# satoken/ractip

Measured on AMD Instinct MI355X. Metric: sequence-pairs/sec (incl. bp+hp+ap DP; host strings in, thresholded matrices out) at n=500, higher is better.
Workload: dtype f64; 1 GPU; synthetic random pairs n=500/500, std::mt19937(12345) stream (BASELINE config 3); scoring=CONTRAfold complementary (708 weights)

## Files before the change

### ractip_amd/csrc/compute.hip

```cpp
#include <hip/hip_runtime.h>

#include <algorithm>
#include <cmath>
#include <cstring>
#include <string>
#include <vector>

#include "ctx.h"
#include "kernels.h"

namespace rh::host {

template <class L, class... Args>
int run_graphed(rh_ctx* c, GraphSlot& g, hipStream_t stream, int k, L launcher, const Args&... args)
{
    const auto launch = [&] { int rc = RH_OK; ((rc = rc ? rc : launcher(c, args)), ...); return rc; };
    if (!c->use_graphs || c->time_cls >= 0) return launch();
    size_t key = 1469598103934665603ull + (sizeof(Args) + ...);
    const auto mix = [&](const void* p, size_t n) { for (size_t q = 0; q < n; q++) key = (key ^ ((const unsigned char*)p)[q]) * 0x100000001b3ull; };
    (mix(&args, sizeof(Args)), ...);
    int *launch_counter = &c->n_launch[k], *far_counter = &c->n_far[k];
    if (!g.exec || g.key != key) {
        if (g.exec) { HIP_TRY(c, hipGraphExecDestroy(g.exec)); g.exec = nullptr; }
        hipGraph_t graph = nullptr;
// ... 4 lines not shown
        if (rc) { if (graph) (void)hipGraphDestroy(graph); return rc; }
        if (e != hipSuccess) { if (graph) (void)hipGraphDestroy(graph); return fail(c, RH_ERR_HIP, "graph capture failed: %s", hipGetErrorString(e)); }
        e = hipGraphInstantiate(&g.exec, graph, nullptr, nullptr, 0);
        (void)hipGraphDestroy(graph);
        if (e != hipSuccess) { g.exec = nullptr; return fail(c, RH_ERR_HIP, "hipGraphInstantiate failed: %s", hipGetErrorString(e)); }
        g.key = key;
        g.launches = *launch_counter - before;
        g.far = *far_counter - far_before;
        *launch_counter = before;
        *far_counter = far_before;
    }
    HIP_TRY(c, hipGraphLaunch(g.exec, stream));
    *launch_counter += g.launches;
    *far_counter += g.far;
    return RH_OK;
}

McLinArgs mc_lin_args(const rh_ctx* c, int phase, const McBatch& B, const LinSet* lin, bool routed)
{
    McLinArgs A;
    A.B = B; A.lin = lin; A.phase = phase;
    A.logz = c->d_mclogz.as<double>(); A.bad = c->d_bad.as<int>();
    A.plan = plan_mc_lin(c, phase, B.nmax);
    if (routed && (!c->small_list.empty() || c->n_short > 0)) {
        A.routed = 1;
        A.small_list = c->d_small_list.as<const int>(); A.n_small = (int)c->small_list.size();
        A.n_sweep = c->d_n_sweep.as<const int>(); A.nmax_sweep = c->nmax_sweep;
        A.n_short = c->d_n_short.as<const int>(); A.nmax_short = c->nmax_short; A.short_count = c->n_short;
        A.plan_sweep = plan_mc_lin(c, phase, A.nmax_sweep);
        A.plan_short = plan_mc_lin(c, phase, A.nmax_short);
    }
    A.pin = xcd_pin(B.ns);
    A.strip_xcd = c->strip_xcd;
    A.f5_jlo = 32;
    A.up_w = c->max_w;
    A.f5_pass = c->f5_pass && f5_pass_fits(B.ld);
    return A;
}

static McVlinArgs mc_vlin_args(const rh_ctx* c, int phase, bool co)
{
    McVlinArgs A;
    A.B = co ? c->co : c->mc; A.phase = phase; A.co = co;
    A.pin = xcd_pin(A.B.ns);
    A.plan = plan_mc_vlin(c, phase, co, A.B.nmax);
    A.d_vlin = c->d_vlin; A.h_vlin = c->h_vlin; A.hplen = c->h_hplen.data(); A.d_hplen = c->d_hplen.as<const double>();
    A.bad = co ? c->d_cobad.as<int>() : c->d_bad.as<int>();
    if (co) {
        const DxBatch& D = c->dx;
        if (A.B.seeded) { A.from = c->mc; A.pair_seq = c->d_pidx.as<const int>(); }
        A.hp = D.hp; A.hp_logz = D.logz; A.hp_stride = D.tab_stride; A.hp_ldd = D.ldd; A.n1max = D.n1max; A.n2max = D.n2max;
        A.cut_min = c->co_cut_min; A.cut_max = c->co_cut_max;
        A.window = c->co_window && c->co_cut_min >= 1 && (phase == 1 || A.B.seeded);
    } else {
        A.logz = c->d_mclogz.as<double>(); A.gaps = c->d_gaps.as<double>(); A.max_w = c->max_w;
        A.acc_wide = c->acc_wide && (size_t)VM_COUNT * A.B.tab_stride * sizeof(double) < ((size_t)1 << 32);
        A.acc_final_t = c->acc_final_t && c->max_w <= 15;
    }
    return A;
}

static DxLinArgs dx_args(const rh_ctx* c)
{
    DxLinArgs A;
    A.X = c->dxl; A.plan = c->plan[2]; A.lz_chunks = c->lz_chunks;
    A.zpart = c->d_zpart.as<double>(); A.zbar = c->d_zbar.as<double>();
// ... 341 lines not shown
```

### ractip_amd/csrc/ctx.h

```cpp
#pragma once
#include <hip/hip_runtime.h>

#include <cassert>
#include <cstdint>
#include <cstring>
#include <string>
#include <type_traits>
#include <vector>

#include "../../include/ractip_hot.h"
#include "batch.h"
#include "batch_request.h"
#include "score_model.h"
#include "lin_model.h"
#include "vienna_model.h"
#include "scale_order.h"

struct rh_ctx;

namespace rh::host {

struct DevBuf {
    void* p = nullptr;
    size_t cap = 0;
// ... 36 lines not shown
};

struct SweepPlan {
    enum Org { kNone, kStrips, kPairs, kLookahead, kDiagonals, kDxStrip8, kDxSweep4, kDxSweepW };
    enum Far { kFarNone, kFarLds, kFarGather, kFarPacked };
    Org org = kNone;
    int W = 0;
    int BS = 0;
    int filt = 0;
    Far far = kFarNone;
    int far2_from = 0;
    int banded = 0;
    int repack2 = 0;
    const char* fine = "";
    const char* far_name = "";
};

static_assert(std::has_unique_object_representations_v<SweepPlan> && std::has_unique_object_representations_v<McBatch>);
static_assert(sizeof(DxLinBatch) == 4 * sizeof(void*) + 6 * sizeof(int) + 3 * sizeof(size_t) + 16 * sizeof(double), "no padding");

struct McLinArgs {
    McBatch B;
    const LinSet* lin;
    double* logz;
    int* bad;
    SweepPlan plan;
    const int* small_list;
    const int* n_sweep;
    const int* n_short;
    SweepPlan plan_sweep, plan_short;
    int routed, n_small, nmax_sweep, short_count, nmax_short;
    int phase, pin, strip_xcd;
    int f5_pass, f5_jlo;
    int up_w, pad_;
    McLinArgs() { std::memset(this, 0, sizeof *this); }
};

struct McVlinArgs {
    McBatch B;
    McBatch from;
    const int* pair_seq;
    SweepPlan plan;
    const VLinModel* d_vlin;
    const VLinModel* h_vlin;
    const double* hplen;
    const double* d_hplen;
    int* bad;
    double* logz;
    double* gaps;
    double* hp;
    double* hp_logz;
    size_t hp_stride;
    int hp_ldd, n1max, n2max;
    int window, cut_min, cut_max;
    int max_w, acc_wide, acc_final_t;
    int phase, pin, co;
    McVlinArgs() { std::memset(this, 0, sizeof *this); }
};

struct DxLinArgs {
    DxLinBatch X;
    SweepPlan plan;
    const DxLinModel* dm;
    const DxLinModel* hm;
    double vdx_s;
    double* zpart;
    double* zbar;
// ... 51 lines not shown
    DxLinModel h_dxlin;
    DevObj<DxLinModel> d_dxlin_r[4];
    DxLinModel h_dxlin_r[4];
    std::vector<int> rescaled_dx;
    DxLinBatch dxl = {};
    size_t dxl_layout = 0;
    size_t dx_bytes = 0;
    bool dxtab_log = false;
    int co_seed = 1;
    int dx_strip = 1;
    int dx_quad = 1;
    int dx_w = 4;
    int last_dx_path = 0;
    int far_mfma = 1;
    int lookahead = 2;
    int strip = 3;
    int far2 = -1;
    int strip_w = 8;
    int small_on = 0;
    std::vector<int> small_list;
    DevBuf d_small_list;
    DevBuf d_n_sweep;
    int nmax_sweep = 0;
    DevBuf d_n_short;
    int n_short = 0, nmax_short = 0;
    int strip_filt = 1;
    bool strip_filt_ok = false;
    int co_cut_min = 0, co_cut_max = 0;
    int co_window = 1;
    int acc_final_t = 1;
    int acc_wide = 1;
    int strip_xcd = 1;
    int f5_pass = 1;
    int far_pk = 1;
    int use_graphs = 1;
    GraphSlot g_in, g_out, g_dx;
    int mode = RH_MODE_AUTO;
    int duplex_mode = RH_MODE_INHERIT;
    int lin_w = 4;
    int lin_w_in = 4;
    int lin_bs = 16;
    int last_path = 0;
    bool last_went_log = false;
    SweepPlan plan[3];
    int max_w = 1;
    int region_acc = 0;
    DevBuf d_acc;
    hipEvent_t acc_ev[2] = {nullptr, nullptr};
    bool acc_timed = false;

    int np = 0, ns = 0;
    std::vector<int> pair_seq;
    std::vector<int> pair_seq_dev;
    bool indexed = false;
    bool has_mc = false, has_dx = false, computed = false;
    std::vector<int> n;
    McBatch mc = {};
    DxBatch dx = {};
    DevBuf d_seq;
    DevBuf d_n;
    DevBuf d_pseq;
    DevBuf d_pn;
    DevBuf d_pidx;
    DevBuf d_mctab;
    DevBuf d_corowp;
    DevBuf d_rowp;
// ... 148 lines not shown
```

### ractip_amd/csrc/kernels.h

```cpp
#pragma once
#include <hip/hip_runtime.h>

#include "../../include/ractip_hot.h"
#include "batch.h"
#include "score_model.h"
#include "lin_model.h"
#include "vienna_model.h"

namespace rh {
__global__ void mc_init(McBatch B);
__global__ void mc_inside_diag(McBatch B, const ScoreModel* __restrict__ M, int d, int pin);
__global__ void mc_outside_diag(McBatch B, const ScoreModel* __restrict__ M, int d, int pin);
__global__ void mc_unpaired(McBatch B, int max_w);
struct AccArgs {
    const LinModel* lin;
    const ScoreModel* score;
    double* scratch;
    int max_w, pad_;
};
constexpr int kAccTile = 64, kAccK = 16;
constexpr size_t acc_scratch_doubles(int ld) { return 3 * (size_t)ld * ld + 2 * 31 * (size_t)ld; }
template <int PATH> __global__ void cf_acc_hrows(McBatch B, AccArgs A);
template <int PATH> __global__ void cf_acc_hcols(McBatch B, AccArgs A);
template <int PATH> __global__ void cf_acc_gaps(McBatch B, AccArgs A);
template <int PATH> __global__ void cf_acc_final(McBatch B, AccArgs A);
template <int PATH> __global__ void cf_acc_sbuild(McBatch B, AccArgs A);
template <int PATH> __global__ void cf_acc_seed(McBatch B, AccArgs A);
template <int PATH> __global__ void cf_acc_link(McBatch B, AccArgs A, int flip);
template <int PATH> __global__ void cf_acc_close(McBatch B, AccArgs A, int j, int flip);
__global__ void dx_sweep_diag(DxBatch B, const ScoreModel* __restrict__ M, int t);
__global__ void dx_logz(DxBatch B, const ScoreModel* __restrict__ M);
__global__ void dx_posterior(DxBatch B);
__global__ void dx_hp_clear_rest(DxBatch B);
__global__ void lin_init(McBatch B, const LinModel* __restrict__ L, int* __restrict__ bad);
template <int W, int BS, int MODE> __global__ void lin_inside_diag(McBatch B, const LinModel* __restrict__ L, int d, double lam_d, int pin);
template <int W, int BS> __global__ void lin_outside_diag(McBatch B, const LinModel* __restrict__ L, int d, int pin, int* __restrict__ bad);
template <int W, int BS> __global__ void lin_outside_pair(McBatch B, const LinModel* __restrict__ L, int d, int khi, int pin, int* __restrict__ bad);
template <int BS> __global__ void lin_far_inside(McBatch B, int D);
template <int BS> __global__ void lin_far_outside(McBatch B, int D);
__global__ void lin_far_inside_mfma(McBatch B, int D);
__global__ void lin_far_outside_mfma(McBatch B, int D);
template <int SWEEP> __global__ void lin_pack_tiles(McBatch B, int Dblk, int outside, int banded);
template <int KD, int W, int FILT> __global__ void lin_inside_strip(McBatch B, const LinModel* __restrict__ L, const double* __restrict__ wT, int d0, double lam_d0, int pin);
template <int KD, int W, int FILT> __global__ void lin_outside_strip(McBatch B, const LinModel* __restrict__ L, const double* __restrict__ wT, int d0, int pin, int* __restrict__ bad);
__global__ void lin_f5i_tail(McBatch B, const LinModel* __restrict__ L, int jlo);
__global__ void lin_f5i_pass(McBatch B, const LinModel* __restrict__ L, int jlo);
void launch_lin_small(const McBatch& B, const LinModel* L, const double* wpad, const int* list, int nlist, int* bad, hipStream_t stream);
__global__ void lin_f5o_head(McBatch B, const LinModel* __restrict__ L, int khi, int klo);
__global__ void lin_f5o_pass(McBatch B, const LinModel* __restrict__ L);
__global__ void lin_far_inside_pk(McBatch B, int D, int l2);
__global__ void lin_far_outside_pk(McBatch B, int D, int l2);
__global__ void lin_far2_inside(McBatch B, int D2, int l2);
__global__ void lin_far2_outside(McBatch B, int D2, int l2);
__global__ void lin_finish(McBatch B, const LinModel* __restrict__ L, double* __restrict__ logz, int* __restrict__ bad);
template <int W> __global__ void dxl_sweep(DxLinBatch B, const DxLinModel* __restrict__ L, int step, int groups);
__global__ void dxl_sweep4(DxLinBatch B, const DxLinModel* __restrict__ L, int step, int groups);
__global__ void dxl_strip8(DxLinBatch B, const DxLinModel* __restrict__ L, int step);
template <bool S20> __global__ void dxvl_sweep4(DxLinBatch B, const VLinModel* __restrict__ L, const VDxLin* __restrict__ D, int step);
template <bool S20> __global__ void dxvl_logz_part(DxLinBatch B, const VLinModel* __restrict__ L, const VDxLin* __restrict__ D, double* __restrict__ zpart,
                               int* __restrict__ cpart, int nchunk);
__global__ void dxvl_logz_final(DxLinBatch B, double s, const double* __restrict__ zpart, const int* __restrict__ cpart, int nchunk,
                                double* __restrict__ zbar, double* __restrict__ logz, int* __restrict__ bad);
constexpr int kLzThreads = 256;
size_t dxl_logz_lds_bytes(int lds);
__global__ void dxl_logz_part(DxLinBatch B, const DxLinModel* __restrict__ L, double* __restrict__ zpart, int* __restrict__ cpart, int nchunk);
__global__ void dxl_logz_final(DxLinBatch B, const DxLinModel* __restrict__ L, const double* __restrict__ zpart, const int* __restrict__ cpart, int nchunk,
                               double* __restrict__ zbar, double* __restrict__ logz, int* __restrict__ bad);
__global__ void dxl_posterior(DxLinBatch B, const double* __restrict__ zbar, int* __restrict__ bad);
__global__ void dxv_sweep_diag(DxBatch B, const ViennaDx* __restrict__ V, int t);
__global__ void dxv_logz(DxBatch B, const ViennaDx* __restrict__ V);
__global__ void dxv_posterior(DxBatch B);
__global__ void mcv_init(McBatch B);
__global__ void mcv_inside_diag(McBatch B, const ViennaDx* __restrict__ V, int d, int pin);
__global__ void mcv_outside_diag(McBatch B, const ViennaDx* __restrict__ V, int d, int pin);
__global__ void mcv_acc_prep(McBatch B, const ViennaDx* __restrict__ V);
__global__ void mcv_acc_hscan(McBatch B, int slot);
__global__ void vlin_acc_prep(McBatch B, const VLinModel* __restrict__ L, const double* __restrict__ hplen);
// ... 71 lines not shown
```

### ractip_amd/csrc/launch_contrafold.hip

```cpp
#include <hip/hip_runtime.h>

#include <algorithm>
#include <cmath>
#include <cstring>
#include <string>
#include <vector>

#include "ctx.h"
#include "f5_stage.h"
#include "kernels.h"

__global__ void log_finish(rh::McBatch B, double* __restrict__ logz)
{
    const int sq = blockIdx.x * blockDim.x + threadIdx.x;
    if (sq < B.ns) logz[sq] = B.f5i[(size_t)sq * B.ld + B.n[sq]];
}

namespace rh::host {

int launch_mc_log(rh_ctx* c, int pin, const McBatch& B, double* logz_out)
{
    hipLaunchKernelGGL(mc_init, dim3((B.ns + 63) / 64), dim3(64), 0, c->s_mc, B);
    for (int d = 0; d <= B.nmax - 1; d++) {
        const int waves = std::max(B.nmax - 1 - d, 0) + 1;
// ... 71 lines not shown
#undef DIAG
#undef STRIP
static const DiagKernels& diag_kernels(int W, int BS) { return row_of(kDiag, [&](const DiagKernels& r) { return r.W == W && r.BS == BS; }); }
static const PairKernels& pair_kernels(int W) { return row_of(kOutsidePair, [&](const PairKernels& r) { return r.W == W; }); }
static const StripKernels& strip_kernels(int W, int filt) { return row_of(kStrip, [&](const StripKernels& r) { return r.W == W && r.filt == filt; }); }
static const LdsKernels& lds_kernels(int BS) { return row_of(kLds, [&](const LdsKernels& r) { return r.BS == BS; }); }

const char* far_name(SweepPlan::Far far, int BS, int phase)
{
    switch (far) {
        case SweepPlan::kFarLds: return phase == 0 ? lds_kernels(BS).in.name : lds_kernels(BS).out.name;
        case SweepPlan::kFarGather: return kFarGather[phase].name;
        case SweepPlan::kFarPacked: return kFarPacked[phase].name;
        default: return "";
    }
}
void far_products(const rh_ctx* c, int phase, int nmax, bool mfma, SweepPlan* P)
{
    const int from = c->far2 >= 0 ? (c->far2 ? 1 : 0) : 384;
    P->far = P->BS == 0 ? SweepPlan::kFarNone : !mfma ? SweepPlan::kFarLds : c->far_pk ? SweepPlan::kFarPacked : SweepPlan::kFarGather;
    P->far2_from = P->far == SweepPlan::kFarPacked && from > 0 && nmax >= from ? from : 0;
    P->far_name = far_name(P->far, P->BS, phase);
}

void far_inside_after(const SweepPass& S, int done)
{
    rh_ctx* c = S.c;
    const McBatch& B = S.B;
    const int D = S.P.BS ? done / S.P.BS + 1 : 0, last_block = S.last_block(), l2 = S.P.far2_from;
    if (S.P.BS == 0 || done % S.P.BS != 0 || D < 4 || D > last_block) return;
    if (S.P.far == SweepPlan::kFarLds) KLAUNCH(c, 1, (lds_kernels(S.P.BS).in.kern), dim3(last_block - D + 1, B.ns), dim3(256), S.st, B, D);
    else if (S.P.far == SweepPlan::kFarGather) KLAUNCH(c, 1, (kFarGather[0].kern), dim3(last_block - D + 1, B.ns), dim3(256), S.st, B, D);
    else {
        KLAUNCH(c, 1, lin_pack_tiles<0>, dim3(B.nb - (D - 2), B.ns, 2), dim3(256), S.st, B, D - 2, 0, (int)S.P.banded);
        if (l2 && (D + 3) % 4 == 0) {
            const int D2 = (D + 3) / 4, last2 = (B.nmax - 1) / 64;
            if (D2 >= 4 && D2 <= last2) KLAUNCH(c, 1, lin_far2_inside, dim3(last2 - D2 + 1, B.ns), dim3(256), S.st, B, D2, l2);
        }
        KLAUNCH(c, 1, (kFarPacked[0].kern), dim3(last_block - D + 1, B.ns), dim3(256), S.st, B, D, l2);
    }
    c->n_launch[S.k]++;
    c->n_far[S.k]++;
}
void far_outside_before(SweepPass& S, int d)
{
    rh_ctx* c = S.c;
    const McBatch& B = S.B;
    const int D = S.P.BS ? (d + 1) / S.P.BS - 1 : 0, last_block = S.last_block(), l2 = S.P.far2_from;
    if (S.P.BS == 0 || (d + 1) % S.P.BS != 0 || D < 0 || D > last_block) return;
    if (S.P.far == SweepPlan::kFarLds) KLAUNCH(c, 3, (lds_kernels(S.P.BS).out.kern), dim3(last_block - D + 1, B.ns, 2), dim3(256), S.st, B, D);
    else if (S.P.far == SweepPlan::kFarGather) KLAUNCH(c, 3, (kFarGather[1].kern), dim3(last_block - D + 1, B.ns, 2), dim3(256), S.st, B, D);
    else {
        if (D + 2 <= last_block) KLAUNCH(c, 3, lin_pack_tiles<1>, dim3(B.nb - (D + 2), B.ns, 1), dim3(256), S.st, B, D + 2, 1, 0);
        if (l2) {
            const int last2 = (B.nmax - 1) / 64;
            for (; S.far2_next >= 0 && 4 * S.far2_next + 3 >= D; S.far2_next--)
                KLAUNCH(c, 3, lin_far2_outside, dim3(last2 - S.far2_next + 1, B.ns, 2), dim3(256), S.st, B, S.far2_next, l2);
        }
        KLAUNCH(c, 3, (kFarPacked[1].kern), dim3(last_block - D + 1, B.ns, 2), dim3(256), S.st, B, D, l2);
    }
    c->n_launch[S.k]++;
    c->n_far[S.k]++;
}
void far_outside_begin(SweepPass& S, int top)
{
    if (S.P.BS == 0) return;
    rh_ctx* c = S.c;
    const McBatch& B = S.B;
    const int last_block = S.last_block(), banded = S.P.banded;
    if (S.P.far == SweepPlan::kFarPacked) {
        S.far2_next = (B.nmax - 1) / 64;
        if (S.P.repack2 && last_block - 1 > 2) KLAUNCH(c, 3, lin_pack_tiles<1>, dim3(B.nb - 2, B.ns, 2), dim3(256), S.st, B, 2, 0, banded);
        for (int Dblk = std::max(2, last_block - 1); Dblk <= last_block; Dblk++)
            KLAUNCH(c, 3, lin_pack_tiles<1>, dim3(B.nb - Dblk, B.ns, 2), dim3(256), S.st, B, Dblk, 0, banded);
    }
    for (int d = (last_block + 1) * S.P.BS - 1; d > top; d -= S.P.BS) far_outside_before(S, d);
}

SweepPlan plan_mc_lin(const rh_ctx* c, int phase, int nmax)
{
    SweepPlan P;
    const int w = phase == 0 ? c->lin_w_in : c->lin_w;
    P.BS = c->lin_bs == 0 || c->lin_bs == 32 ? c->lin_bs : 16;
    P.W = w == 16 ? 16 : (w == 4 && P.BS == 16 ? 4 : 8);
    const bool all_orgs = P.W == 4 && P.BS == 16, strips_ok = c->far_pk && c->far_mfma && c->lin_bs == 16 && nmax >= kStripMinN;
    const bool strips_on = (c->strip & (phase == 0 ? 1 : 2)) && strips_ok, strips = all_orgs && strips_on;
    const StripKernels& strip = strip_kernels(c->strip_w, c->strip_w == 8 && c->strip_filt && c->strip_filt_ok);
    const DiagKernels& diag = diag_kernels(P.W, P.BS);
    bool mfma = P.BS == 16 && c->far_mfma;
    P.org = SweepPlan::kDiagonals;
    P.fine = phase == 0 ? diag.in.name : diag.out.name;
    if (strips) {
        P.org = SweepPlan::kStrips;
        P.W = strip.W;
        P.filt = strip.filt;
    } else if (phase == 0 && all_orgs && c->lookahead == 2) {
        P.org = SweepPlan::kPairs;
        P.fine = kInsidePair.name;
        mfma = true;
    } else if (phase == 0 && all_orgs && c->lookahead) {
        P.org = SweepPlan::kLookahead;
        P.fine = kInsideAhead[0].name;
    } else if (phase == 1 && mfma && (P.W == 4 || P.W == 8) && c->lookahead == 2) {
        P.org = SweepPlan::kPairs;
        P.fine = pair_kernels(P.W).out.name;
    }
    far_products(c, phase, nmax, mfma, &P);
// ... 29 lines not shown
                (A.pin && A.strip_xcd) ? 2 : A.pin);
        c->n_launch[0]++;
        far_inside_after(S, d0 + KD);
    }
    if (A.f5_pass) hipLaunchKernelGGL(lin_f5i_pass, dim3(B.ns), dim3(256), f5_pass_lds(B.ld, 0), S.st, B, A.lin->d, A.f5_jlo);
    else hipLaunchKernelGGL(lin_f5i_tail, dim3(B.ns), dim3(256), 0, S.st, B, A.lin->d, A.f5_jlo);
}
static void inside_diagonals(const SweepPass& S, const McLinArgs& A, bool ahead)
{
    const InsideDiagK full = diag_kernels(S.P.W, S.P.BS).in.kern;
    for (int d = 0; d <= S.B.nmax - 1; d++) {
        const int groups = (std::max(S.B.nmax - 1 - d, 0) + 63) / 64 + 1;
        const bool odd = ahead && (d & 1);
        KLAUNCH(S.c, 0, (!ahead ? full : kInsideAhead[odd].kern), seq_grid(A.pin, S.B.ns, groups), dim3(odd ? 64 : 64 * S.P.W), S.st, S.B, A.lin->d, d,
                std::exp(-A.lin->h.s * d), A.pin);
        S.c->n_launch[0]++;
        far_inside_after(S, d + 1);
    }
}

static void outside_strips(SweepPass& S, const McLinArgs& A)
{
    rh_ctx* c = S.c;
    const McBatch& B = S.B;
    constexpr int KD = 8, GS = 64 - (KD - 1);
    const auto strip = strip_kernels(S.P.W, S.P.filt).out.kern;
    const int d0_top = (B.nmax - 2) | (KD - 1);
    far_outside_begin(S, d0_top);
    if (A.f5_pass) hipLaunchKernelGGL(lin_f5o_pass, dim3(B.ns), dim3(256), f5_pass_lds(B.ld, 1), S.st, B, A.lin->d);
    else hipLaunchKernelGGL(lin_f5o_head, dim3(B.ns), dim3(256), 0, S.st, B, A.lin->d, B.nmax - 1, 1);
    for (int d0 = d0_top; d0 >= KD - 1; d0 -= KD) {
        far_outside_before(S, d0);
        const int groups = (B.nmax - 1 - (d0 - (KD - 1)) + GS - 1) / GS;
        KLAUNCH(c, 2, strip, seq_grid(A.pin, B.ns, groups), dim3(64 * S.P.W), S.st, B, A.lin->d, A.lin->wT, d0, (A.pin && A.strip_xcd) ? 2 : A.pin, A.bad);
        c->n_launch[1]++;
    }
}
static void outside_pairs(SweepPass& S, const McLinArgs& A)
{
    const auto pair = pair_kernels(S.P.W).out.kern;
    far_outside_begin(S, S.B.nmax - 2);
    for (int d = (S.B.nmax - 2) | 1; d >= 0; d -= 2) {
        for (int r = d; r >= d - 1 && r >= 0; r--) far_outside_before(S, r);
        const int ncol = S.B.nmax - 1 - d + 1;
        const int groups = std::max(1, (ncol - 1 + 62) / 63) + 1;
        KLAUNCH(S.c, 2, pair, seq_grid(A.pin, S.B.ns, groups), dim3(64 * S.P.W), S.st, S.B, A.lin->d, d, d, A.pin, A.bad);
        S.c->n_launch[1]++;
    }
}
static void outside_diagonals(SweepPass& S, const McLinArgs& A)
{
    const auto diag = diag_kernels(S.P.W, S.P.BS).out.kern;
    far_outside_begin(S, S.B.nmax - 2);
    for (int d = S.B.nmax - 2; d >= 0; d--) {
        far_outside_before(S, d);
        const int groups = (S.B.nmax - 1 - d + 63) / 64 + 1;
        KLAUNCH(S.c, 2, diag, seq_grid(A.pin, S.B.ns, groups), dim3(64 * S.P.W), S.st, S.B, A.lin->d, d, A.pin, A.bad);
        S.c->n_launch[1]++;
    }
}

int launch_mc_lin(rh_ctx* c, const McLinArgs& A)
{
    const McBatch& BR = A.B;
    const int phase = A.phase;
    const auto sweep = [&](const McBatch& B, const SweepPlan& Q) {
        SweepPass S{c, Q, B, c->s_mc, phase};
// ... 75 lines not shown
```

### ractip_amd/csrc/mccaskill_far.hip

```cpp
#include <hip/hip_runtime.h>

#include "batch.h"
#include "lin_model.h"
#include "kernels.h"

namespace rh {

static_assert((int)VL_FM1 == (int)L_FM1 && (int)VL_FM == (int)L_FM && (int)VL_FM2O == (int)L_FM2O && (int)VL_FM2F == (int)L_FM2F &&
                  (int)VL_FMOF == (int)L_FMOF && (int)VL_FM1OF == (int)L_FM1OF,
              "LinTable and VLinTable disagree on a slot of the block products: FM1, FM, FM2O, FM2F, FMOF, FM1OF");

namespace {

__device__ __forceinline__ double cellv(const double* __restrict__ T, int ld, int n, int x, int y)
{
    return (x >= 1 && x <= y && y <= n - 1) ? T[(size_t)(y - x) * ld + x] : 0.0;
}

template <int BS, bool TR>
__device__ __forceinline__ void load_chunk(double (*dst)[BS + 1], const double* __restrict__ T, int ld, int n, int x0, int y0)
{
    const int u = threadIdx.x % BS;
    constexpr int DPP = 256 / BS;
    for (int dd = threadIdx.x / BS; dd < 2 * BS - 1; dd += DPP) {
// ... 176 lines not shown
    const int I = blockIdx.x, J = I + D;
    if (J * 16 > n - 1) return;
    const int w = threadIdx.x >> 6;
    const int ld = B.ld;
    double* __restrict__ tab = B.tab + (size_t)sq * B.seq_stride;
    const double* __restrict__ fm1 = tab + (size_t)L_FM1 * B.tab_stride;
    const double* __restrict__ fm = tab + (size_t)L_FM * B.tab_stride;
    const double* __restrict__ fm2o = tab + (size_t)L_FM2O * B.tab_stride;
    d4 acc = {0.0, 0.0, 0.0, 0.0};
    if (blockIdx.z == 0) {
        for (int K = w; K <= I - 2; K += 4) {
            load_chunk16_wave<true>(A[w], fm1, ld, n, K * 16, I * 16);
            load_chunk16_wave<false>(Bm[w], fm2o, ld, n, K * 16, J * 16);
            acc = mfma_chunk(A[w], Bm[w], acc);
        }
        reduce_store(red, acc, tab + (size_t)L_FMOF * B.tab_stride, ld, n, I * 16, J * 16);
    } else {
        const int last = (n - 1) / 16;
        for (int K = J + 2 + w; K <= last; K += 4) {
            load_chunk16_wave<false>(A[w], fm2o, ld, n, I * 16, K * 16);
            load_chunk16_wave<true>(Bm[w], fm, ld, n, J * 16, K * 16);
            acc = mfma_chunk(A[w], Bm[w], acc);
        }
        reduce_store(red, acc, tab + (size_t)L_FM1OF * B.tab_stride, ld, n, I * 16, J * 16);
    }
}

enum PkCopy { PK_FM1_A = 0, PK_FM1_B, PK_FM_A, PK_FM_B, PK_FM2O_A, PK_FM2O_B };
__device__ __forceinline__ size_t pk_tile(int nb, int P, int Q) { return ((size_t)P * nb - (size_t)P * (P - 1) / 2 + (Q - P)) * 256; }

template <int SWEEP>
__global__ __launch_bounds__(256) void lin_pack_tiles(McBatch B, int Dblk, int outside, int banded)
{
    __shared__ double T[16][17];
    const int sq = blockIdx.y;
    const int n = B.n[sq];
    const int P = blockIdx.x, Q = P + Dblk;
    if (Q >= B.nb || Q * 16 > n - 1) return;
    const int slot = outside ? L_FM2O : (blockIdx.z == 0 ? L_FM1 : L_FM);
    const int copy = outside ? PK_FM2O_A : (blockIdx.z == 0 ? PK_FM1_A : PK_FM_A);
    const double* __restrict__ src = B.tab + (size_t)sq * B.seq_stride + (size_t)slot * B.tab_stride;
    {
        const int u = threadIdx.x & 15;
#pragma unroll
        for (int pass = 0; pass < 2; pass++) {
            const int v = u + (threadIdx.x >> 4) + 16 * pass - 15;
            if (v >= 0 && v < 16) T[u][v] = (banded && !outside && Dblk == 2 && v < u) ? 0.0 : cellv(src, B.ld, n, P * 16 + u, Q * 16 + v);
        }
    }
    __syncthreads();
    double* __restrict__ dst = B.pk + ((size_t)sq * kPkCopies + copy) * B.pk_stride + pk_tile(B.nb, P, Q);
    const int s = threadIdx.x & 3, l = threadIdx.x >> 2, r = l & 15, q = l >> 4;
    dst[threadIdx.x] = T[r][4 * s + q];
    dst[B.pk_stride + threadIdx.x] = T[4 * s + q][r];
}

__device__ __forceinline__ d4 mfma4(d4 a, d4 b, d4 acc)
{
#pragma unroll
    for (int s = 0; s < 4; s++) acc = __builtin_amdgcn_mfma_f64_16x16x4f64(a[s], b[s], acc, 0, 0, 0);
    return acc;
}

template <class TA, class TB>
__device__ __forceinline__ d4 pk_loop(const double* __restrict__ pa, const double* __restrict__ pb, int k_lo, int k_hi, TA ta, TB tb,
                                      d4 acc = d4{0.0, 0.0, 0.0, 0.0})
{
    const int w = threadIdx.x >> 6, lane = threadIdx.x & 63;
    int K = k_lo + w;
    for (; K + 4 <= k_hi; K += 8) {
        const d4 a0 = *(const d4*)(pa + ta(K) + lane * 4), b0 = *(const d4*)(pb + tb(K) + lane * 4);
        const d4 a1 = *(const d4*)(pa + ta(K + 4) + lane * 4), b1 = *(const d4*)(pb + tb(K + 4) + lane * 4);
        acc = mfma4(a0, b0, acc);
        acc = mfma4(a1, b1, acc);
    }
    if (K <= k_hi) {
        const d4 a0 = *(const d4*)(pa + ta(K) + lane * 4), b0 = *(const d4*)(pb + tb(K) + lane * 4);
        acc = mfma4(a0, b0, acc);
    }
    return acc;
}


__device__ __forceinline__ bool one_strand_tile(const McBatch& B, int sq, bool inside, int lo_i, int hi_j)
{
    if (!B.cut || (inside && !B.seeded)) return false;
    const int cut = B.cut[sq];
// ... 143 lines not shown
```

### ractip_amd/csrc/mccaskill_strip.hip

```cpp
#include <hip/hip_runtime.h>

#include <type_traits>
#include <utility>

#include "batch.h"
#include "dev_util.h"
#include "f5_stage.h"
#include "lin_model.h"
#include "kernels.h"

namespace rh {

namespace {

template <int V> using IC = std::integral_constant<int, V>;
template <class F, int... Is> __device__ __forceinline__ void static_for_impl(F&& f, std::integer_sequence<int, Is...>) { (f(IC<Is>{}), ...); }
template <int N, class F> __device__ __forceinline__ void static_for(F&& f) { static_for_impl(f, std::make_integer_sequence<int, N>{}); }

}

#ifdef RH_STAMPS
__device__ unsigned long long g_stamps[16];
#define RH_STAMP(k) do { const unsigned long long t_ = __builtin_amdgcn_s_memtime(); st_acc_[k] += t_ - t_prev_; t_prev_ = t_; \
        if ((k) == 8 && threadIdx.x == 0) { for (int k_ = 0; k_ < 15; k_++) if (st_acc_[k_]) atomicAdd(&g_stamps[k_], st_acc_[k_]); atomicAdd(&g_stamps[15], 1ull); } } while (0)
// ... 817 lines not shown
                }
                if (t < kF5ParkT) {
#pragma unroll
                    for (int e = 2; e < kF5Blk; e++)
                        if (t <= e - 2 && exists(r, e)) park[f5_park_slot(q, e, t)] = row[e];
                }
            }
            lds_barrier();
        }
#pragma unroll
        for (int e = 0; e < kF5Blk; e++) {
            if (e < ne) {
                const int k = k0 - e;
                double a = acc[e];
                if (e >= 2 && t <= e - 2) {
                    a = 0.0;
                    for (int q = 0; k + 2 + t + 256 * q <= n; q++) a = f5_term(f5s[k + 2 + t + 256 * q], park[f5_park_slot(q, e, t)], a);
                }
                a = wsum(a);
                if (lane == 0) red[(e & 1) * 4 + w] = a;
                lds_barrier();
                const double* r = red + (e & 1) * 4;
                prev = f5_entry(prev, r[0], r[1], r[2], r[3], w_eu, w_ep2);
                if (t == 0) f5s[k] = prev;
            }
        }
        lds_barrier();
        if (t < ne) f5o[k0 - t] = f5s[k0 - t];
    }
}

template <int KD, int W, int FILT>
__global__ __launch_bounds__(64 * W, (W >= 8 ? 4 : 2)) void lin_outside_strip(McBatch B, const LinModel* __restrict__ L, const double* __restrict__ wT, int d0,
                                                                              int pin, int* __restrict__ bad)
{
    using P = OutStripPlan<KD, W>;
    constexpr int GS = P::GS, NM = P::NM, CD = P::CD, CA = P::CA, CE = P::CE, CS = P::CS, PADL = P::PADL;
    constexpr int NSL = KD / W;
    constexpr int TS = P::TS, KH = KD * TS / W;
    static_assert(KD % W == 0 && KD <= 8 && W % TS == 0 && KD % (W / TS) == 0 && (NM + 1) % W == 0, "8 terms per end and term set, 32/W staged rows per wavefront and region");
    __shared__ double lds[P::SZ];
    constexpr bool FACT = FILT != 0 && W == 8 && KD == 8;
    __shared__ double fw[FACT ? 160 : 1];
    int sq = pin ? blockIdx.x : blockIdx.y, slot = pin ? blockIdx.y : blockIdx.x;
    if (pin == 2) {
        const unsigned lin = blockIdx.x + blockIdx.y * gridDim.x, t = lin >> 3;
        slot = (int)(t % gridDim.y);
        sq = (int)(t / gridDim.y) * 8 + (int)(lin & 7);
    }
    if (sq >= B.ns) return;
    const int n = B.n[sq];
    const int w = __builtin_amdgcn_readfirstlane(threadIdx.x >> 6), lane = threadIdx.x & 63;
    const int wt = w % TS, kb = (w / TS) * KH;
    const int ld = B.ld;
    const size_t ts = B.tab_stride;
    const uint8_t* __restrict__ s = B.seq + (size_t)sq * B.lds;
    double* __restrict__ tab = B.tab + (size_t)sq * B.seq_stride;
    const double* __restrict__ f5i = B.f5i + (size_t)sq * ld;
    double* __restrict__ f5o = B.f5o + (size_t)sq * ld;
    const int dlow = d0 - (KD - 1);
    const int ncell_max = n - 1 - dlow > 0 ? n - 1 - dlow : 0;
    const int ngroup = (ncell_max + GS - 1) / GS;
    if (slot >= ngroup) return;

#ifdef RH_STAGGER
    {
        const unsigned lin = blockIdx.x + blockIdx.y * gridDim.x;
// ... 421 lines not shown
        SFCO[K * CS + PADL + lane] = fco; SFCOX[K * CS + PADL + lane] = fco * p_tjbx[SL];
        fco_s[SL] = fco;
    };
    RH_STAMPO(6);
#define RH_SLOT(T)                                                                                  \
    if constexpr (T < KD) {                                                                         \
        if (w == T % W) fin(IC<T>{});                                                               \
        if constexpr (T >= 1 && T + 1 < KD)                                                         \
            static_for<KD>([&](auto KC) {                                                           \
                constexpr int K = decltype(KC)::value;                                              \
                if constexpr (K > T) { if (w == K % W) addrow(IC<(T >= 1 ? T - 1 : 0)>{}, KC); }    \
            });                                                                                     \
        if constexpr (T + 1 < KD) lds_barrier();                                                    \
    }
    RH_SLOT(0) RH_SLOT(1) RH_SLOT(2) RH_SLOT(3) RH_SLOT(4) RH_SLOT(5) RH_SLOT(6) RH_SLOT(7)
#undef RH_SLOT
    RH_STAMPO(7);
#pragma unroll
    for (int sl = 0; sl < NSL; sl++) {
        const int K = w + W * sl, d = d0 - K;
        const bool v = i >= 1 && d >= 0 && i <= n - 1 - d;
        double p = fco_s[sl] * p_fc[sl] * r_z;
        if (v && lane >= KD - 1 && (!(p == p) || p > 1e300)) { atomicOr(&bad[sq], 1); p = 0.0; }
        p = p > 1.0 ? 1.0 : (p < 0.0 ? 0.0 : p);
        if (!(p == p)) p = 0.0;
        PART[(K * 3) * 64 + lane] = p;
    }
    lds_barrier();
    if (lane >= KD - 1 && i >= 1) {
#pragma unroll 1
        for (int r = w; r < 5 * KD; r += W) {
            const int tb = r / KD, k = r - tb * KD, d = d0 - k;
            const int slot_of[5] = {L_FM2O, L_FMO, L_FM1O, L_FCO, L_FCOX};
            if (d >= 0 && i <= n - 1 - d) tab[slot_of[tb] * ts + (size_t)d * ld + i] = SFM2O[r * CS + PADL + lane];
        }
    }
    for (int t = threadIdx.x; t < 64 * KD; t += 64 * W) {
        const int c = t / KD, k = t - c * KD, ii = i0 + c, d = d0 - k;
        if (c >= KD - 1 && ii >= 1 && d >= 0 && ii <= n - 1 - d)
            B.bp[(size_t)sq * B.tri_stride + tri_off(n, ii) + (ii + d + 1)] = PART[(k * 3) * 64 + c];
    }
    RH_STAMPO(8);
}

template __global__ void lin_inside_strip<8, 4, 0>(McBatch, const LinModel*, const double*, int, double, int);
template __global__ void lin_inside_strip<8, 8, 0>(McBatch, const LinModel*, const double*, int, double, int);
template __global__ void lin_inside_strip<8, 8, 1>(McBatch, const LinModel*, const double*, int, double, int);
template __global__ void lin_outside_strip<8, 4, 0>(McBatch, const LinModel*, const double*, int, int, int*);
template __global__ void lin_outside_strip<8, 8, 0>(McBatch, const LinModel*, const double*, int, int, int*);
template __global__ void lin_outside_strip<8, 8, 1>(McBatch, const LinModel*, const double*, int, int, int*);

}
```

### ractip_amd/csrc/rh_api.hip

```cpp
#include <hip/hip_runtime.h>

#include <dlfcn.h>

#include <algorithm>
#include <cstdarg>
#include <cstdio>
#include <cstdlib>
#include <cstring>
#include <string>
#include <vector>

#include "ctx.h"
#include "kernels.h"

using namespace rh;
using namespace rh::host;

__global__ void collect_logz(const double* __restrict__ mc_logz, const int* __restrict__ idx, DxBatch D, double* __restrict__ out)
{
    const int p = blockIdx.x * blockDim.x + threadIdx.x;
    if (p >= D.np) return;
    out[3 * p + 0] = mc_logz[idx[2 * p]];
    out[3 * p + 1] = mc_logz[idx[2 * p + 1]];
    out[3 * p + 2] = D.logz[p];
// ... 64 lines not shown
}
int fetch_hp(rh_ctx* c, int p, double* out, double* logz)
{
    const int n1 = c->n[seq_of(c, p, 0)], n2 = c->n[seq_of(c, p, 1)];
    if (out)
        HIP_TRY(c, hipMemcpy2D(out, sizeof(double) * (n2 + 1), c->d_hp.as<const double>() + (size_t)p * c->dx.tab_stride,
                               sizeof(double) * c->dx.ldd, sizeof(double) * (n2 + 1), n1 + 1, hipMemcpyDeviceToHost));
    if (logz) HIP_TRY(c, hipMemcpy(logz, c->d_logz.as<const double>() + p, sizeof(double), hipMemcpyDeviceToHost));
    return RH_OK;
}

enum EnvKind { ENV_INT, ENV_FLAG , ENV_NOT , ENV_4OR8 , ENV_DOUBLE };
struct EnvSwitch {
    const char* name;
    EnvKind kind;
    int Ctx::*field;
    double Ctx::*dfield = nullptr;
};
const EnvSwitch kEnvSwitches[] = {
    {"RH_LIN_W", ENV_INT, &Ctx::lin_w},        {"RH_LIN_W", ENV_INT, &Ctx::lin_w_in},
    {"RH_LIN_W_IN", ENV_INT, &Ctx::lin_w_in},
    {"RH_LIN_BS", ENV_INT, &Ctx::lin_bs},
    {"RH_NO_GRAPH", ENV_NOT, &Ctx::use_graphs},
    {"RH_FAR_MFMA", ENV_FLAG, &Ctx::far_mfma},
    {"RH_FAR_PK", ENV_FLAG, &Ctx::far_pk},
    {"RH_LOOKAHEAD", ENV_INT, &Ctx::lookahead},
    {"RH_STRIP", ENV_INT, &Ctx::strip},
    {"RH_STRIP_W", ENV_4OR8, &Ctx::strip_w},
    {"RH_STRIP_FILT", ENV_FLAG, &Ctx::strip_filt},
    {"RH_SMALL", ENV_FLAG, &Ctx::small_on},
    {"RH_FAR2", ENV_INT, &Ctx::far2},
    {"RH_STRIP_XCD", ENV_INT, &Ctx::strip_xcd},
    {"RH_F5_PASS", ENV_FLAG, &Ctx::f5_pass},
    {"RH_ACC_WIDE", ENV_INT, &Ctx::acc_wide},
    {"RH_ACC_FINAL_T", ENV_INT, &Ctx::acc_final_t},
    {"RH_CO_WINDOW", ENV_INT, &Ctx::co_window},
    {"RH_SCALE_LADDER", ENV_INT, &Ctx::scale_ladder},
    {"RH_SCALE_MEMORY", ENV_INT, &Ctx::scale_memory},
    {"RH_PAIR_HELPER", ENV_INT, &Ctx::pair_helper},
    {"RH_CO_SEED", ENV_INT, &Ctx::co_seed},
    {"RH_DX_W", ENV_INT, &Ctx::dx_w},
    {"RH_DX_QUAD", ENV_FLAG, &Ctx::dx_quad},
    {"RH_DX_STRIP", ENV_INT, &Ctx::dx_strip},
    {"RH_VDX_S", ENV_DOUBLE, nullptr, &Ctx::vdx_s},
};

}

extern "C" {

static rh_ctx* create_ctx(int device, int model, const char* param_file, const char* defaults_file, int use_bl, int semantics);

rh_ctx* rh_create(int device, int model, const char* param_file) { return create_ctx(device, model, param_file, nullptr, 1, 0); }
rh_ctx* rh_create_vienna(int device, const char* defaults_file, int use_bl_param, const char* param_file, int semantics)
{
    return create_ctx(device, RH_MODEL_VIENNA_BL, param_file, defaults_file, use_bl_param, semantics);
}
int rh_vienna_semantics(const rh_ctx* c) { return c ? c->vienna_sem : RH_ERR_ARG; }

static rh_ctx* create_ctx(int device, int model, const char* param_file, const char* defaults_file, int use_bl, int semantics)
{
    if (model != RH_MODEL_CONTRAFOLD && model != RH_MODEL_VIENNA_BL) {
        fail(nullptr, RH_ERR_UNSUPPORTED, "unknown model %d", model);
        return nullptr;
    }
    int ndev = 0;
// ... 582 lines not shown
```

Baseline: 12430 pairs/s.

## Pack runs of far tiles per block and skip redundant outside-strip table stores

The tile-packing kernel now handles a run of eight consecutive tiles per block. All loads are issued up front into registers with wavefront-coalesced addressing, and the tiles are then written out of a larger shared-memory buffer, which cuts the block count and per-block overhead. Separately, the outside strip kernel skips writing back the diagonals of some table slots that later stages apparently do not read. The full store is kept behind an env flag, and it is forced on when region accumulation is active. This relies on the skipped diagonals being truly unused, and the packing kernel now needs more shared memory and registers per block.

Result: no change. 12550 pairs/s, median of 6 (+1.0%).

```diff
diff --git a/ractip_amd/csrc/compute.hip b/ractip_amd/csrc/compute.hip
--- a/ractip_amd/csrc/compute.hip
+++ b/ractip_amd/csrc/compute.hip
@@ -60,6 +60,7 @@
     }
     A.pin = xcd_pin(B.ns);
     A.strip_xcd = c->strip_xcd;
+    A.strip_store_all = c->strip_store_all || c->region_acc;
     A.f5_jlo = 32;
     A.up_w = c->max_w;
     A.f5_pass = c->f5_pass && f5_pass_fits(B.ld);
diff --git a/ractip_amd/csrc/ctx.h b/ractip_amd/csrc/ctx.h
--- a/ractip_amd/csrc/ctx.h
+++ b/ractip_amd/csrc/ctx.h
@@ -92,7 +92,8 @@
     int routed, n_small, nmax_sweep, short_count, nmax_short;
     int phase, pin, strip_xcd;
     int f5_pass, f5_jlo;
-    int up_w, pad_;
+    int up_w;
+    int strip_store_all;
     McLinArgs() { std::memset(this, 0, sizeof *this); }
 };
 
@@ -210,6 +211,7 @@
     int acc_wide = 1;
     int strip_xcd = 1;
     int f5_pass = 1;
+    int strip_store_all = 0;
     int far_pk = 1;
     int use_graphs = 1;
     GraphSlot g_in, g_out, g_dx;
diff --git a/ractip_amd/csrc/kernels.h b/ractip_amd/csrc/kernels.h
--- a/ractip_amd/csrc/kernels.h
+++ b/ractip_amd/csrc/kernels.h
@@ -40,9 +40,11 @@
 template <int BS> __global__ void lin_far_outside(McBatch B, int D);
 __global__ void lin_far_inside_mfma(McBatch B, int D);
 __global__ void lin_far_outside_mfma(McBatch B, int D);
+constexpr int kPackRun = 8;
+constexpr int pack_runs(int tiles) { return (tiles + kPackRun - 1) / kPackRun; }
 template <int SWEEP> __global__ void lin_pack_tiles(McBatch B, int Dblk, int outside, int banded);
 template <int KD, int W, int FILT> __global__ void lin_inside_strip(McBatch B, const LinModel* __restrict__ L, const double* __restrict__ wT, int d0, double lam_d0, int pin);
-template <int KD, int W, int FILT> __global__ void lin_outside_strip(McBatch B, const LinModel* __restrict__ L, const double* __restrict__ wT, int d0, int pin, int* __restrict__ bad);
+template <int KD, int W, int FILT> __global__ void lin_outside_strip(McBatch B, const LinModel* __restrict__ L, const double* __restrict__ wT, int d0, int pin, int* __restrict__ bad, int store_all);
 __global__ void lin_f5i_tail(McBatch B, const LinModel* __restrict__ L, int jlo);
 __global__ void lin_f5i_pass(McBatch B, const LinModel* __restrict__ L, int jlo);
 void launch_lin_small(const McBatch& B, const LinModel* L, const double* wpad, const int* list, int nlist, int* bad, hipStream_t stream);
diff --git a/ractip_amd/csrc/launch_contrafold.hip b/ractip_amd/csrc/launch_contrafold.hip
--- a/ractip_amd/csrc/launch_contrafold.hip
+++ b/ractip_amd/csrc/launch_contrafold.hip
@@ -127,7 +127,7 @@
     if (S.P.far == SweepPlan::kFarLds) KLAUNCH(c, 1, (lds_kernels(S.P.BS).in.kern), dim3(last_block - D + 1, B.ns), dim3(256), S.st, B, D);
     else if (S.P.far == SweepPlan::kFarGather) KLAUNCH(c, 1, (kFarGather[0].kern), dim3(last_block - D + 1, B.ns), dim3(256), S.st, B, D);
     else {
-        KLAUNCH(c, 1, lin_pack_tiles<0>, dim3(B.nb - (D - 2), B.ns, 2), dim3(256), S.st, B, D - 2, 0, (int)S.P.banded);
+        KLAUNCH(c, 1, lin_pack_tiles<0>, dim3(pack_runs(B.nb - (D - 2)), B.ns, 2), dim3(256), S.st, B, D - 2, 0, (int)S.P.banded);
         if (l2 && (D + 3) % 4 == 0) {
             const int D2 = (D + 3) / 4, last2 = (B.nmax - 1) / 64;
             if (D2 >= 4 && D2 <= last2) KLAUNCH(c, 1, lin_far2_inside, dim3(last2 - D2 + 1, B.ns), dim3(256), S.st, B, D2, l2);
@@ -146,7 +146,7 @@
     if (S.P.far == SweepPlan::kFarLds) KLAUNCH(c, 3, (lds_kernels(S.P.BS).out.kern), dim3(last_block - D + 1, B.ns, 2), dim3(256), S.st, B, D);
     else if (S.P.far == SweepPlan::kFarGather) KLAUNCH(c, 3, (kFarGather[1].kern), dim3(last_block - D + 1, B.ns, 2), dim3(256), S.st, B, D);
     else {
-        if (D + 2 <= last_block) KLAUNCH(c, 3, lin_pack_tiles<1>, dim3(B.nb - (D + 2), B.ns, 1), dim3(256), S.st, B, D + 2, 1, 0);
+        if (D + 2 <= last_block) KLAUNCH(c, 3, lin_pack_tiles<1>, dim3(pack_runs(B.nb - (D + 2)), B.ns, 1), dim3(256), S.st, B, D + 2, 1, 0);
         if (l2) {
             const int last2 = (B.nmax - 1) / 64;
             for (; S.far2_next >= 0 && 4 * S.far2_next + 3 >= D; S.far2_next--)
@@ -165,9 +165,9 @@
     const int last_block = S.last_block(), banded = S.P.banded;
     if (S.P.far == SweepPlan::kFarPacked) {
         S.far2_next = (B.nmax - 1) / 64;
-        if (S.P.repack2 && last_block - 1 > 2) KLAUNCH(c, 3, lin_pack_tiles<1>, dim3(B.nb - 2, B.ns, 2), dim3(256), S.st, B, 2, 0, banded);
+        if (S.P.repack2 && last_block - 1 > 2) KLAUNCH(c, 3, lin_pack_tiles<1>, dim3(pack_runs(B.nb - 2), B.ns, 2), dim3(256), S.st, B, 2, 0, banded);
         for (int Dblk = std::max(2, last_block - 1); Dblk <= last_block; Dblk++)
-            KLAUNCH(c, 3, lin_pack_tiles<1>, dim3(B.nb - Dblk, B.ns, 2), dim3(256), S.st, B, Dblk, 0, banded);
+            KLAUNCH(c, 3, lin_pack_tiles<1>, dim3(pack_runs(B.nb - Dblk), B.ns, 2), dim3(256), S.st, B, Dblk, 0, banded);
     }
     for (int d = (last_block + 1) * S.P.BS - 1; d > top; d -= S.P.BS) far_outside_before(S, d);
 }
@@ -263,7 +263,8 @@
     for (int d0 = d0_top; d0 >= KD - 1; d0 -= KD) {
         far_outside_before(S, d0);
         const int groups = (B.nmax - 1 - (d0 - (KD - 1)) + GS - 1) / GS;
-        KLAUNCH(c, 2, strip, seq_grid(A.pin, B.ns, groups), dim3(64 * S.P.W), S.st, B, A.lin->d, A.lin->wT, d0, (A.pin && A.strip_xcd) ? 2 : A.pin, A.bad);
+        KLAUNCH(c, 2, strip, seq_grid(A.pin, B.ns, groups), dim3(64 * S.P.W), S.st, B, A.lin->d, A.lin->wT, d0, (A.pin && A.strip_xcd) ? 2 : A.pin, A.bad,
+                A.strip_store_all);
         c->n_launch[1]++;
     }
 }
diff --git a/ractip_amd/csrc/mccaskill_far.hip b/ractip_amd/csrc/mccaskill_far.hip
--- a/ractip_amd/csrc/mccaskill_far.hip
+++ b/ractip_amd/csrc/mccaskill_far.hip
@@ -232,27 +232,46 @@
 template <int SWEEP>
 __global__ __launch_bounds__(256) void lin_pack_tiles(McBatch B, int Dblk, int outside, int banded)
 {
-    __shared__ double T[16][17];
-    const int sq = blockIdx.y;
-    const int n = B.n[sq];
-    const int P = blockIdx.x, Q = P + Dblk;
-    if (Q >= B.nb || Q * 16 > n - 1) return;
+    constexpr int R = kPackRun, NC = 16 * R / 64, NL = 8 * NC;
+    constexpr int TST = 16 * 17 + 1;
+    static_assert((16 * R) % 64 == 0, "a span is whole wavefront loads");
+    __shared__ double T[R * TST];
+    const int sq = blockIdx.y;
+    const int n = B.n[sq];
+    const int P0 = blockIdx.x * R;
+    if (P0 + Dblk >= B.nb || (P0 + Dblk) * 16 > n - 1) return;
     const int slot = outside ? L_FM2O : (blockIdx.z == 0 ? L_FM1 : L_FM);
     const int copy = outside ? PK_FM2O_A : (blockIdx.z == 0 ? PK_FM1_A : PK_FM_A);
     const double* __restrict__ src = B.tab + (size_t)sq * B.seq_stride + (size_t)slot * B.tab_stride;
+    const int w = threadIdx.x >> 6, lane = threadIdx.x & 63;
+    const bool mask = banded && !outside && Dblk == 2;
     {
-        const int u = threadIdx.x & 15;
-#pragma unroll
-        for (int pass = 0; pass < 2; pass++) {
-            const int v = u + (threadIdx.x >> 4) + 16 * pass - 15;
-            if (v >= 0 && v < 16) T[u][v] = (banded && !outside && Dblk == 2 && v < u) ? 0.0 : cellv(src, B.ld, n, P * 16 + u, Q * 16 + v);
+        double val[NL];
+#pragma unroll
+        for (int k = 0; k < NL; k++) {
+            const int dl = w - 15 + 4 * (k / NC), c = (k % NC) * 64 + lane;
+            const int u = c & 15, v = u + dl, x = P0 * 16 + c, d = Dblk * 16 + dl;
+            const bool ok = (dl <= 15) & (v >= 0) & (v < 16) & (x >= 1) & (d >= 0) & (x + d <= n - 1) & !(mask & (v < u));
+            val[k] = src[ok ? (size_t)d * B.ld + x : (size_t)0];
+            if (!ok) val[k] = 0.0;
+        }
+#pragma unroll
+        for (int k = 0; k < NL; k++) {
+            const int dl = w - 15 + 4 * (k / NC), c = (k % NC) * 64 + lane;
+            const int u = c & 15, v = u + dl;
+            if (dl <= 15 && v >= 0 && v < 16) T[(c >> 4) * TST + u * 17 + v] = val[k];
         }
     }
     __syncthreads();
-    double* __restrict__ dst = B.pk + ((size_t)sq * kPkCopies + copy) * B.pk_stride + pk_tile(B.nb, P, Q);
     const int s = threadIdx.x & 3, l = threadIdx.x >> 2, r = l & 15, q = l >> 4;
-    dst[threadIdx.x] = T[r][4 * s + q];
-    dst[B.pk_stride + threadIdx.x] = T[4 * s + q][r];
+#pragma unroll
+    for (int t = 0; t < R; t++) {
+        const int P = P0 + t, Q = P + Dblk;
+        if (Q >= B.nb || Q * 16 > n - 1) break;
+        double* __restrict__ dst = B.pk + ((size_t)sq * kPkCopies + copy) * B.pk_stride + pk_tile(B.nb, P, Q);
+        dst[threadIdx.x] = T[t * TST + r * 17 + 4 * s + q];
+        dst[B.pk_stride + threadIdx.x] = T[t * TST + (4 * s + q) * 17 + r];
+    }
 }
 
 __device__ __forceinline__ d4 mfma4(d4 a, d4 b, d4 acc)
diff --git a/ractip_amd/csrc/mccaskill_strip.hip b/ractip_amd/csrc/mccaskill_strip.hip
--- a/ractip_amd/csrc/mccaskill_strip.hip
+++ b/ractip_amd/csrc/mccaskill_strip.hip
@@ -873,7 +873,7 @@
 
 template <int KD, int W, int FILT>
 __global__ __launch_bounds__(64 * W, (W >= 8 ? 4 : 2)) void lin_outside_strip(McBatch B, const LinModel* __restrict__ L, const double* __restrict__ wT, int d0,
-                                                                              int pin, int* __restrict__ bad)
+                                                                              int pin, int* __restrict__ bad, int store_all)
 {
     using P = OutStripPlan<KD, W>;
     constexpr int GS = P::GS, NM = P::NM, CD = P::CD, CA = P::CA, CE = P::CE, CS = P::CS, PADL = P::PADL;
@@ -1361,6 +1361,8 @@
         for (int r = w; r < 5 * KD; r += W) {
             const int tb = r / KD, k = r - tb * KD, d = d0 - k;
             const int slot_of[5] = {L_FM2O, L_FMO, L_FM1O, L_FCO, L_FCOX};
+            const int first = tb == 1 ? KD - 1 : (tb == 2 || tb == 3) ? KD - 2 : 0;
+            if (!store_all && k < first) continue;
             if (d >= 0 && i <= n - 1 - d) tab[slot_of[tb] * ts + (size_t)d * ld + i] = SFM2O[r * CS + PADL + lane];
         }
     }
@@ -1375,8 +1377,8 @@
 template __global__ void lin_inside_strip<8, 4, 0>(McBatch, const LinModel*, const double*, int, double, int);
 template __global__ void lin_inside_strip<8, 8, 0>(McBatch, const LinModel*, const double*, int, double, int);
 template __global__ void lin_inside_strip<8, 8, 1>(McBatch, const LinModel*, const double*, int, double, int);
-template __global__ void lin_outside_strip<8, 4, 0>(McBatch, const LinModel*, const double*, int, int, int*);
-template __global__ void lin_outside_strip<8, 8, 0>(McBatch, const LinModel*, const double*, int, int, int*);
-template __global__ void lin_outside_strip<8, 8, 1>(McBatch, const LinModel*, const double*, int, int, int*);
-
-}
+template __global__ void lin_outside_strip<8, 4, 0>(McBatch, const LinModel*, const double*, int, int, int*, int);
+template __global__ void lin_outside_strip<8, 8, 0>(McBatch, const LinModel*, const double*, int, int, int*, int);
+template __global__ void lin_outside_strip<8, 8, 1>(McBatch, const LinModel*, const double*, int, int, int*, int);
+
+}
diff --git a/ractip_amd/csrc/rh_api.hip b/ractip_amd/csrc/rh_api.hip
--- a/ractip_amd/csrc/rh_api.hip
+++ b/ractip_amd/csrc/rh_api.hip
@@ -120,6 +120,7 @@
     {"RH_FAR2", ENV_INT, &Ctx::far2},
     {"RH_STRIP_XCD", ENV_INT, &Ctx::strip_xcd},
     {"RH_F5_PASS", ENV_FLAG, &Ctx::f5_pass},
+    {"RH_STRIP_STORE_ALL", ENV_FLAG, &Ctx::strip_store_all},
     {"RH_ACC_WIDE", ENV_INT, &Ctx::acc_wide},
     {"RH_ACC_FINAL_T", ENV_INT, &Ctx::acc_final_t},
     {"RH_CO_WINDOW", ENV_INT, &Ctx::co_window},
```
